# zifeo/distributed-sgd

Hardware: NVIDIA H100
Metric: sgd_samples_per_sec (higher is better)
Workload: dtype f64

## Files before the change

### distributed_sgd_b200/csrc/dsgd_fixed.cuh

```cuda
#pragma once
#include <cuda_runtime.h>
#include <stdint.h>

namespace dsgd {

constexpr int kAccStride = 16;
constexpr int kAccLimbs = 5;
constexpr int kAccWords = 2 * kAccLimbs + 1;
static_assert(kAccWords + 1 <= kAccStride, "acc_read loads the accumulator and one pad word");
__device__ __forceinline__ void red_add_u64(unsigned long long *p, unsigned long long v) {
  asm volatile("red.relaxed.gpu.global.add.u64 [%0], %1;" ::"l"(p), "l"(v) : "memory");
}
template <class Put>
__device__ __forceinline__ void acc_cut(double a, Put &&put) {
  double F[kAccLimbs - 1];
#pragma unroll
  for (int i = 0; i < kAccLimbs - 1; ++i) F[i] = floor(a * __longlong_as_double((1023ll + 40 * i) << 52));
  put(kAccLimbs - 1, F[0]);
#pragma unroll
  for (int i = 1; i < kAccLimbs - 1; ++i) put(kAccLimbs - 1 - i, F[i] - F[i - 1] * 0x1p40);
  put(0, rint(a * 0x1p160) - F[kAccLimbs - 2] * 0x1p40);
}
__device__ __forceinline__ void acc_push_one(unsigned long long *limbs, unsigned long long *ovf, double v) {
  if (!(fabs(v) < 4503599627370496.0)) {
    red_add_u64(ovf, 1ull);
    return;
  }
  const bool neg = v < 0.0;
  acc_cut(fabs(v), [&](int k, double limb) {
    if (limb != 0.0) {
      const unsigned long long u = (unsigned long long)(long long)limb;
      red_add_u64(limbs + k, neg ? (0ull - u) : u);
    }
  });
}
__device__ __forceinline__ void acc_push(unsigned long long *acc, double sd, double sn) {
  acc_push_one(acc, acc + 2 * kAccLimbs, sd);
  acc_push_one(acc + kAccLimbs, acc + 2 * kAccLimbs, sn);
}
__device__ __forceinline__ double acc_limb(unsigned long long q, int k) {
  return (double)(long long)q * __longlong_as_double((long long)(1023 - 160 + 40 * (k % kAccLimbs)) << 52);
}
__device__ __forceinline__ void acc_read(const unsigned long long *acc, int lane, double &sd, double &sn) {
  unsigned long long q0 = 0, q1 = 0;
  if (lane < (kAccWords + 1) / 2)
    asm volatile("ld.relaxed.gpu.global.v2.u64 {%0, %1}, [%2];" : "=l"(q0), "=l"(q1) : "l"(acc + 2 * lane) : "memory");
  const double lo = acc_limb(q0, 2 * lane), hi = acc_limb(q1, 2 * lane + 1), pair = lo + hi;
  const double s01 = __shfl_sync(0xffffffffu, pair, 0), s23 = __shfl_sync(0xffffffffu, pair, 1);
  const double s4 = __shfl_sync(0xffffffffu, lo, 2), n0 = __shfl_sync(0xffffffffu, hi, 2);
  const double n12 = __shfl_sync(0xffffffffu, pair, 3), n34 = __shfl_sync(0xffffffffu, pair, 4);
  sd = (s01 + s23) + s4;
  sn = (n0 + n12) + n34;
  if (__any_sync(0xffffffffu, lane == kAccWords / 2 && q0 != 0)) {
    sd = __longlong_as_double(0x7ff8000000000000ll);
    sn = sd;
  }
}

constexpr int kLossLimbs = kAccLimbs + 1;
constexpr int kLossAccWords = kLossLimbs + 1;
constexpr unsigned long long kLimbMask = (1ull << 40) - 1;
__device__ __forceinline__ void acc_carry(unsigned long long (&q)[kLossLimbs]) {
#pragma unroll
  for (int i = 0; i < kLossLimbs - 1; ++i) {
    q[i + 1] += q[i] >> 40;
    q[i] &= kLimbMask;
  }
}
__device__ __forceinline__ void acc_add_local(unsigned long long (&lim)[kLossLimbs], unsigned long long &ovf, double v) {
  if (!(v >= 0.0 && v < 4503599627370496.0)) { ++ovf; return; }
  acc_cut(v, [&](int k, double limb) { lim[k] += (unsigned long long)(long long)limb; });
  acc_carry(lim);
}
__device__ __forceinline__ void acc_flush_local(unsigned long long *acc, const unsigned long long (&lim)[kLossLimbs],
                                                unsigned long long ovf) {
#pragma unroll
  for (int i = 0; i < kLossLimbs; ++i)
    if (lim[i]) red_add_u64(acc + i, lim[i]);
  if (ovf) red_add_u64(acc + kLossLimbs, ovf);
}
__device__ __forceinline__ double acc_value(const unsigned long long *acc) {
  if (acc[kLossLimbs] != 0ull) return __longlong_as_double(0x7ff8000000000000ll);
  unsigned long long q[kLossLimbs];
#pragma unroll
  for (int i = 0; i < kLossLimbs; ++i) q[i] = acc[i];
  acc_carry(q);
  double s = (double)q[kLossLimbs - 1] * 0x1p40;
#pragma unroll
  for (int i = kLossLimbs - 2; i >= 0; --i) s += (double)q[i] * __longlong_as_double((long long)(1023 - 160 + 40 * i) << 52);
  return s;
}

}
```

### distributed_sgd_b200/csrc/dsgd_persistent.cuh

```cuda
#pragma once
#include <cuda_runtime.h>
#include <stdint.h>

#include "dsgd_fixed.cuh"
#include "dsgd_kernels.cuh"

namespace dsgd {

constexpr int kMaxWorld = 8;

struct PersistParams {
  const uint32_t *rp16;
  const uint2 *pairs;
  const int8_t *label;
  const int32_t *samples;
  int64_t n_steps;
  int32_t batch;
  int32_t dim;
  double *wbuf[2];
  double *gbuf[3];
  double2 *rec[3];
  const double *d;
  unsigned long long *acc;
  unsigned *hinge;
  double *losses;
  double *w_out;
  float *w32_out;
  double *scal;
  unsigned *bar;
  int *abort_flag;
  double lambda, lr, k_den;
  long long timeout_cycles;
  long long *tl;
  int world, rank;
  int64_t step_base;
  unsigned long long *xval[kMaxWorld];
  unsigned long long *xbm[kMaxWorld];
  int xstride, xwords;
  unsigned long long *llw[2];
  unsigned long long *xstats;
  double *avg;
};
static_assert(sizeof(PersistParams) <= 4000, "kernel parameter space is 4 KB");

__device__ __forceinline__ uint32_t smem_u32(const void *p) { return (uint32_t)__cvta_generic_to_shared(p); }
__device__ __forceinline__ void mbar_init(uint64_t *b, unsigned count) {
  asm volatile("mbarrier.init.shared::cta.b64 [%0], %1;" ::"r"(smem_u32(b)), "r"(count) : "memory");
}
__device__ __forceinline__ void mbar_expect_tx(uint64_t *b, unsigned bytes) {
  asm volatile("mbarrier.arrive.expect_tx.shared::cta.b64 _, [%0], %1;" ::"r"(smem_u32(b)), "r"(bytes) : "memory");
}
__device__ __forceinline__ void mbar_arrive(uint64_t *b) {
  asm volatile("mbarrier.arrive.shared::cta.b64 _, [%0];" ::"r"(smem_u32(b)) : "memory");
}
__device__ __forceinline__ void bulk_g2s(void *dst, const void *src, unsigned bytes, uint64_t *b) {
  asm volatile("cp.async.bulk.shared::cluster.global.mbarrier::complete_tx::bytes [%0], [%1], %2, [%3];" ::"r"(
                   smem_u32(dst)),
               "l"(src), "r"(bytes), "r"(smem_u32(b))
               : "memory");
}
__device__ __forceinline__ bool mbar_try_wait(uint64_t *b, unsigned parity) {
  unsigned ok;
  asm volatile(
      "{\n\t.reg .pred p;\n\tmbarrier.try_wait.parity.shared::cta.b64 p, [%1], %2;\n\tselp.u32 %0, 1, 0, p;\n\t}"
      : "=r"(ok)
      : "r"(smem_u32(b)), "r"(parity)
      : "memory");
  return ok != 0;
}
__device__ __forceinline__ void mbar_wait(uint64_t *b, unsigned parity, int *abort_flag, long long timeout) {
  if (mbar_try_wait(b, parity)) return;
  const long long t0 = clock64();
  unsigned spins = 0;
  while (!mbar_try_wait(b, parity)) {
    if ((++spins & 255u) == 0u && (clock64() - t0 > timeout || *(volatile int *)abort_flag)) {
      *(volatile int *)abort_flag = 1;
      return;
    }
  }
}
__device__ __forceinline__ unsigned ld_relaxed_gpu(const unsigned *p) {
  unsigned v;
  asm volatile("ld.relaxed.gpu.global.u32 %0, [%1];" : "=r"(v) : "l"(p) : "memory");
  return v;
}
__device__ __forceinline__ void red_release_gpu_add(unsigned *p, unsigned v) {
  asm volatile("red.release.gpu.global.add.u32 [%0], %1;" ::"l"(p), "r"(v) : "memory");
}
__device__ __forceinline__ unsigned atom_acq_rel_gpu_add(unsigned *p, unsigned v) {
  unsigned old;
  asm volatile("atom.acq_rel.gpu.global.add.u32 %0, [%1], %2;" : "=r"(old) : "l"(p), "r"(v) : "memory");
  return old;
}
__device__ __forceinline__ void st_relaxed_gpu(unsigned *p, unsigned v) {
  asm volatile("st.relaxed.gpu.global.u32 [%0], %1;" ::"l"(p), "r"(v) : "memory");
}
__device__ __forceinline__ void fence_acq_rel_gpu() { asm volatile("fence.acq_rel.gpu;" ::: "memory"); }
__device__ __forceinline__ void named_bar_sync(int id, int n_threads) {
  asm volatile("bar.sync %0, %1;" ::"r"(id), "r"(n_threads) : "memory");
}
__device__ __forceinline__ long long global_ns() {
  long long t;
  asm volatile("mov.u64 %0, %%globaltimer;" : "=l"(t));
  return t;
}

__device__ __forceinline__ void ll_store(unsigned long long *dst, double v, unsigned tag) {
  const unsigned long long bits = (unsigned long long)__double_as_longlong(v);
  const unsigned long long w0 = (bits & 0xffffffffull) | ((unsigned long long)tag << 32);
  const unsigned long long w1 = (bits >> 32) | ((unsigned long long)tag << 32);
  asm volatile("st.relaxed.sys.global.v2.u64 [%0], {%1, %2};" ::"l"(dst), "l"(w0), "l"(w1) : "memory");
}
__device__ __forceinline__ bool ll_try_load(const unsigned long long *src, unsigned tag, double &v) {
  unsigned long long w0, w1;
  asm volatile("ld.relaxed.sys.global.v2.u64 {%0, %1}, [%2];" : "=l"(w0), "=l"(w1) : "l"(src) : "memory");
  if ((unsigned)(w0 >> 32) != tag || (unsigned)(w1 >> 32) != tag) return false;
  v = __longlong_as_double((long long)((w0 & 0xffffffffull) | (w1 << 32)));
  return true;
}
__device__ __forceinline__ void ll_store32(unsigned long long *dst, unsigned v, unsigned tag) {
  const unsigned long long w = (unsigned long long)v | ((unsigned long long)tag << 32);
  asm volatile("st.relaxed.sys.global.u64 [%0], %1;" ::"l"(dst), "l"(w) : "memory");
}
__device__ __forceinline__ bool ll_try_load32(const unsigned long long *src, unsigned tag, unsigned &v) {
  unsigned long long w;
  asm volatile("ld.relaxed.sys.global.u64 %0, [%1];" : "=l"(w) : "l"(src) : "memory");
  v = (unsigned)w;
  return (unsigned)(w >> 32) == tag;
}

__device__ __forceinline__ double apply_update(double wv, double graw, double c, bool add_c, double k_den, double lr) {
  double v = filt(graw);
  if (v != 0.0) {
    if (add_c) v = filt(v + c);
    if (v != 0.0) {
      const double mean = (k_den == 1.0) ? v : filt(v / k_den);
      const double step = filt(mean * lr);
      wv = filt(wv - step);
    }
  }
  return wv;
}

__device__ __forceinline__ bool grid_barrier_arrive_wait(unsigned *bar, unsigned target, int *abort_flag, long long timeout) {
  red_release_gpu_add(bar, 1u);
  const long long t0 = clock64();
  unsigned spins = 0;
  bool ok = true;
  while ((int)(ld_relaxed_gpu(bar) - target) < 0) {
    if ((++spins & 1023u) == 0u && (clock64() - t0 > timeout || *(volatile int *)abort_flag)) {
      *(volatile int *)abort_flag = 1;
      ok = false;
      break;
    }
  }
  return ok;
}

constexpr int kChunkPairs = 128;
constexpr uint32_t kChunkGlobal = 1u << 31;
constexpr int kMaxRowsPerCta = 32;

template <int kMaxChunks>
struct StageMeta {
  int n_rows;
  int n_chunks;
  int n_multi;
  int n_pairs;
  int row_y[kMaxRowsPerCta];
  uint32_t row_b[kMaxRowsPerCta];
  int row_len[kMaxRowsPerCta];
  short row_first[kMaxRowsPerCta];
  short row_nch[kMaxRowsPerCta];
  uint32_t ch_off[kMaxChunks];
  short ch_n[kMaxChunks];
  short ch_row[kMaxChunks];
  double part[kMaxChunks];
};

template <int kCons, int kUpd, int kStages, int kStagePairs, int kMaxChunks>
struct PersistSmem {
  uint2 ring[kStages][kStagePairs];
  StageMeta<kMaxChunks> meta[kStages];
  uint64_t full[kStages];
  uint64_t empty[kStages];
  uint64_t c_bar[2];
  uint64_t u_bar;
  double red[kCons + kUpd][2];
  double c_val[2];
  double nrm_val[2];
  unsigned hinge_acc;
  int ok;
  long long tl_warp[kCons + kUpd];
};

#define DSGD_TL(slot_)                                                                        \
  do {                                                                                        \
    if (p.tl && blockIdx.x == 0 && lane == 0 && t < 256) p.tl[t * 16 + (slot_)] = clock64(); \
  } while (0)
constexpr int kTlSteps = 4, kTlFirst = 100, kTlCtas = 160, kTlPerCta = 4;
constexpr int kTlWords = 256 * 16 + kTlSteps * kTlCtas * kTlPerCta;

struct FetchLocal {
  const double2 *R;
  uint64_t *cbar;
  unsigned cpar;
  const double *cval;
  int *abort_flag;
  long long timeout;
  double k_den, lr;
  double c = 0.0;
  bool add_c = false, have_c = false, good = true;
  __device__ __forceinline__ void need_c() {
    if (!have_c) {
      mbar_wait(cbar, cpar, abort_flag, timeout);
      c = *(volatile const double *)cval;
      add_c = (c != 0.0) && (fabs(c) > kEps);
      have_c = true;
    }
  }
  __device__ __forceinline__ void get4(const uint2 (&pr)[4], double (&wv)[4]) {
    double2 r[4];
#pragma unroll
    for (int u = 0; u < 4; ++u) {
      r[u] = make_double2(0.0, 0.0);
      if (pr[u].y << 1) r[u] = __ldcg(&R[pr[u].x]);
    }
    need_c();
#pragma unroll
    for (int u = 0; u < 4; ++u) wv[u] = apply_update(r[u].x, r[u].y, c, add_c, k_den, lr);
  }
  __device__ __forceinline__ double get1(uint32_t col) {
    need_c();
    const double2 r = __ldcg(&R[col]);
    return apply_update(r.x, r.y, c, add_c, k_den, lr);
  }
};
struct FetchLL {
  const unsigned long long *LW;
  unsigned tag;
  int *abort_flag;
  long long timeout;
  bool good = true;
  __device__ __forceinline__ void spin(const unsigned long long *src, double &v) {
    unsigned spins = 0;
    const long long t0 = clock64();
    while (!ll_try_load(src, tag, v)) {
      if ((++spins & 255u) == 0u && (clock64() - t0 > timeout || *(volatile int *)abort_flag)) {
        *(volatile int *)abort_flag = 1;
        good = false;
        v = 0.0;
        break;
      }
    }
  }
  __device__ __forceinline__ void get4(const uint2 (&pr)[4], double (&wv)[4]) {
    unsigned pend = 0;
#pragma unroll
    for (int u = 0; u < 4; ++u) {
      wv[u] = 0.0;
      if (pr[u].y << 1) pend |= 1u << u;
    }
    unsigned spins = 0;
    const long long t0 = clock64();
    while (pend) {
      unsigned long long w0[4], w1[4];
#pragma unroll
      for (int u = 0; u < 4; ++u) {
        w0[u] = 0ull; w1[u] = 0ull;
        if (pend & (1u << u))
          asm volatile("ld.relaxed.sys.global.v2.u64 {%0, %1}, [%2];" : "=l"(w0[u]), "=l"(w1[u]) : "l"(LW + 2 * (size_t)pr[u].x) : "memory");
      }
#pragma unroll
      for (int u = 0; u < 4; ++u)
        if ((pend & (1u << u)) && (unsigned)(w0[u] >> 32) == tag && (unsigned)(w1[u] >> 32) == tag) {
          wv[u] = __longlong_as_double((long long)((w0[u] & 0xffffffffull) | (w1[u] << 32)));
          pend &= ~(1u << u);
        }
      if (pend && (++spins & 63u) == 0u && (clock64() - t0 > timeout || *(volatile int *)abort_flag)) {
        *(volatile int *)abort_flag = 1;
        good = false;
        pend = 0;
      }
    }
  }
  __device__ __forceinline__ double get1(uint32_t col) {
    double v;
    spin(LW + 2 * (size_t)col, v);
    return v;
  }
};

template <int kCons, int kMaxChunks, class Fetch>
__device__ __forceinline__ unsigned consume_stage(StageMeta<kMaxChunks> &mt, const uint2 *ring, const uint2 *pairs, double *gbase,
                                                  const int gstride, Fetch &fetch, int warp, int lane, long long *tl) {
  const int n_ch = mt.n_chunks;
  unsigned hinge = 0;
  for (int c = warp; c < n_ch; c += kCons) {
    const uint32_t off = mt.ch_off[c];
    const int n = mt.ch_n[c];
    const uint2 *src = (off & kChunkGlobal) ? (pairs + (off & ~kChunkGlobal)) : (ring + off);
    uint2 pr[4];
    double wv[4];
#pragma unroll
    for (int u = 0; u < 4; ++u) {
      const int k = u * 32 + lane;
      pr[u] = (k < n) ? src[k] : make_uint2(0u, 0u);
    }
    fetch.get4(pr, wv);
    double acc = 0.0;
#pragma unroll
    for (int u = 0; u < 4; ++u) acc += filt(filt((double)__uint_as_float(pr[u].y)) * wv[u]);
    if (tl && lane == 0 && c == warp) tl[2] = clock64();
    acc = warp_sum(acc);
    if (tl && lane == 0 && c == warp) tl[4] = clock64();
    {
      const int row1 = mt.ch_row[c];
      if (mt.row_nch[row1] == 1) {
        const int yi = mt.row_y[row1];
        const double y = (double)yi;
        if (lane == 0) hinge += (unsigned)(1 - yi * pred_of(acc));
        if (!(y * acc < 0.0)) {
#pragma unroll
          for (int u = 0; u < 4; ++u) {
            const double gvv = filt(filt((double)__uint_as_float(pr[u].y)) * y);
            if (gvv != 0.0) red_add_f64(gbase + (size_t)gstride * pr[u].x, gvv);
          }
        }
        continue;
      }
    }
    if (lane == 0) mt.part[c] = acc;
  }
  if (mt.n_multi > 0) {
    named_bar_sync(2, kCons * 32);
    for (int c = warp; c < n_ch; c += kCons) {
      const int row = mt.ch_row[c];
      const int first = mt.row_first[row], nch = mt.row_nch[row];
      if (nch == 1) continue;
      double dot = 0.0;
      for (int i = 0; i < nch; ++i) dot += mt.part[first + i];
      const int yi = mt.row_y[row];
      const double y = (double)yi;
      if (c == first && lane == 0) hinge += (unsigned)(1 - yi * pred_of(dot));
      if (!(y * dot < 0.0)) {
        const uint32_t off = mt.ch_off[c];
        const int n = mt.ch_n[c];
        const uint2 *src = (off & kChunkGlobal) ? (pairs + (off & ~kChunkGlobal)) : (ring + off);
        for (int k = lane; k < n; k += 32) {
          const uint2 pr = src[k];
          const double gvv = filt(filt((double)__uint_as_float(pr.y)) * y);
          if (gvv != 0.0) red_add_f64(gbase + (size_t)gstride * pr.x, gvv);
        }
      }
    }
  }
  for (int m = warp; m < mt.n_rows; m += kCons) {
    const int nch = mt.row_nch[m];
    if (nch == 0) {
      if (lane == 0) hinge += 1u;
    } else if (nch < 0) {
      const uint2 *grow = pairs + (size_t)mt.row_b[m] * 2;
      const int len = mt.row_len[m];
      double acc = 0.0;
      for (int k = lane; k < len; k += 32) {
        const uint2 pr = __ldg(&grow[k]);
        acc += filt(filt((double)__uint_as_float(pr.y)) * fetch.get1(pr.x));
      }
      const double dot = warp_sum(acc);
      const int yi = mt.row_y[m];
      const double y = (double)yi;
      if (lane == 0) hinge += (unsigned)(1 - yi * pred_of(dot));
      if (!(y * dot < 0.0))
        for (int k = lane; k < len; k += 32) {
          const uint2 pr = __ldg(&grow[k]);
          const double gvv = filt(filt((double)__uint_as_float(pr.y)) * y);
          if (gvv != 0.0) red_add_f64(gbase + (size_t)gstride * pr.x, gvv);
        }
    }
  }
  return hinge;
}

template <int kCons, int kUpd, int kStages, int kStagePairs, int kMaxChunks, bool kMulti, bool kAvg>
__global__ void __launch_bounds__((kCons + kUpd + 1) * 32, 1) k_sync_persistent(const PersistParams p) {
  using Smem = PersistSmem<kCons, kUpd, kStages, kStagePairs, kMaxChunks>;
  extern __shared__ __align__(128) unsigned char smem_raw[];
  Smem &sm = *reinterpret_cast<Smem *>(smem_raw);

  const int lane = threadIdx.x & 31;
  const int warp = threadIdx.x >> 5;
  const bool is_cons = warp < kCons;
  const bool is_upd = warp >= kCons && warp < kCons + kUpd;
  const int G = gridDim.x;
  const int B = p.batch;
  const int64_t S = p.n_steps;
  constexpr int kSyncThreads = (kCons + kUpd) * 32;
  const int n_r = (B > (int)blockIdx.x) ? (B - 1 - (int)blockIdx.x) / G + 1 : 0;

  if (threadIdx.x == 0) {
    for (int s = 0; s < kStages; ++s) {
      mbar_init(&sm.full[s], 1u);
      mbar_init(&sm.empty[s], (unsigned)kCons);
    }
    mbar_init(&sm.c_bar[0], 1u);
    mbar_init(&sm.c_bar[1], 1u);
    mbar_init(&sm.u_bar, (unsigned)(kMulti ? kCons + kUpd : kUpd));
    sm.c_val[0] = 0.0;
    sm.nrm_val[0] = 0.0;
    sm.hinge_acc = 0u;
    sm.ok = 1;
  }
  asm volatile("fence.mbarrier_init.release.cluster;" ::: "memory");
  __syncthreads();
  if (threadIdx.x == 0) mbar_arrive(&sm.c_bar[0]);

  if (!is_cons && !is_upd) {
    auto load_id = [&](int64_t t) -> int32_t {
      return (t < S && lane < n_r) ? __ldg(&p.samples[t * B + blockIdx.x + lane * G]) : -1;
    };
    uint32_t b0 = 0, e0 = 0, b1 = 0, e1 = 0;
    int y0 = 0, y1 = 0;
    auto load_win = [&](int32_t id, uint32_t &b, uint32_t &e, int &y) {
      b = 0u; e = 0u; y = 0;
      if (id >= 0) {
        b = __ldg(&p.rp16[id]);
        e = __ldg(&p.rp16[id + 1]);
        y = (int)__ldg(&p.label[id]);
      }
    };
    load_win(load_id(0), b0, e0, y0);
    load_win(load_id(1), b1, e1, y1);
    int32_t id_next = load_id(2);
    for (int64_t t = 0; t < S; ++t) {
      const int st = (int)t & (kStages - 1);
      if (t >= kStages) {
        mbar_wait(&sm.empty[st], (unsigned)(((t / kStages) - 1) & 1), p.abort_flag, p.timeout_cycles);
        if (*(volatile int *)p.abort_flag) return;
      }
      auto &mt = sm.meta[st];
      const int len = (lane < n_r) ? (int)(e0 - b0) * 2 : 0;
      const int nch = (len + kChunkPairs - 1) / kChunkPairs;
      int ps = len, cs = nch;
#pragma unroll
      for (int o = 1; o < 32; o <<= 1) {
        const int a = __shfl_up_sync(0xffffffffu, ps, o), c2 = __shfl_up_sync(0xffffffffu, cs, o);
        if (lane >= o) { ps += a; cs += c2; }
      }
      const int my_pair = ps - len, my_chunk = cs - nch;
      const bool listed = (my_chunk + nch) <= kMaxChunks;
      const bool in_ring = listed && (my_pair + len) <= kStagePairs;
      if (lane < n_r) {
        mt.row_y[lane] = y0;
        mt.row_b[lane] = b0;
        mt.row_len[lane] = len;
        mt.row_first[lane] = (short)my_chunk;
        mt.row_nch[lane] = (short)(listed ? nch : -1);
        if (listed) {
          for (int c = 0; c < nch; ++c) {
            const int n = min(kChunkPairs, len - c * kChunkPairs);
            mt.ch_off[my_chunk + c] = in_ring ? (uint32_t)(my_pair + c * kChunkPairs)
                                              : (kChunkGlobal | (b0 * 2u + (uint32_t)(c * kChunkPairs)));
            mt.ch_n[my_chunk + c] = (short)n;
            mt.ch_row[my_chunk + c] = (short)lane;
          }
        }
      }
      const unsigned my_bytes = (lane < n_r && in_ring) ? (unsigned)len * 8u : 0u;
      const unsigned ring_bytes = __reduce_add_sync(0xffffffffu, my_bytes);
      const int listed_chunks = __reduce_max_sync(0xffffffffu, (lane < n_r && listed) ? (my_chunk + nch) : 0);
      const unsigned multi = __ballot_sync(0xffffffffu, lane < n_r && listed && nch > 1);
      if (lane == 31) mt.n_pairs = ps;
      if (lane == 0) {
        mt.n_rows = n_r;
        mt.n_chunks = listed_chunks;
        mt.n_multi = __popc(multi);
      }
      __syncwarp();
      if (lane == 0) {
        if (ring_bytes) mbar_expect_tx(&sm.full[st], ring_bytes);
        else mbar_arrive(&sm.full[st]);
      }
      __syncwarp();
      if (my_bytes) bulk_g2s(&sm.ring[st][my_pair], p.pairs + (size_t)b0 * 2, my_bytes, &sm.full[st]);
      b0 = b1; e0 = e1; y0 = y1;
      load_win(id_next, b1, e1, y1);
      id_next = load_id(t + 3);
    }
    return;
  }

  const double lr = p.lr;
  const int64_t base = kMulti ? p.step_base : 0;
  unsigned phase = 0;
  const int n_upd = G * kUpd * 32;
  const int u0 = blockIdx.x * kUpd * 32 + ((int)threadIdx.x - kCons * 32);
  const int K = p.world, me = p.rank;
  const int slice = ((p.dim + 1 + G - 1) / G + 31) & ~31;
  const int j_col = blockIdx.x * slice + (int)threadIdx.x;
  const bool col_act = kMulti && (int)threadIdx.x < slice && j_col <= p.dim;
  const int col_word = j_col >> 5;
  unsigned long long st_val = 0, st_bm = 0;
  constexpr int kUpdCols = 2;
  double wreg[kUpdCols], dreg[kUpdCols];
  double areg[kUpdCols];
  int ttl[kUpdCols];
  bool gnz[kUpdCols];
#pragma unroll
  for (int i = 0; i < kUpdCols; ++i) {
    wreg[i] = dreg[i] = 0.0;
    areg[i] = 0.0;
    ttl[i] = 0;
    gnz[i] = false;
    if constexpr (!kMulti) {
      const int j = u0 + i * n_upd;
      if (is_upd && j < p.dim) {
        wreg[i] = __ldcg(&p.rec[2][j].x);
        dreg[i] = __ldg(&p.d[j]);
        if constexpr (kAvg) areg[i] = p.avg[j];
      }
    }
  }
  if constexpr (kMulti) {
    if (col_act && j_col < p.dim) {
      wreg[0] = __ldcg(&p.wbuf[0][j_col]);
      dreg[0] = __ldg(&p.d[j_col]);
      if constexpr (kAvg) areg[0] = p.avg[j_col];
    }
  }

  int gi_prev = (int)((base + 2) % 3), gi_cur = (int)(base % 3), gi_next = (int)((base + 1) % 3);
  int ti_prev = 2, ti_cur = 0, ti_next = 1;
  for (int64_t T = base; T <= base + S; ++T) {
    const int64_t t = T - base;
    const bool first = (t == 0), last = (t == S);
    const double *Gprev = p.gbuf[gi_prev];
    double *Gcur = p.gbuf[gi_cur];
    double *Gzero = p.gbuf[gi_next];
    const unsigned long long *acc_prev = p.acc + (size_t)ti_prev * kAccStride;
    unsigned long long *acc_cur = p.acc + (size_t)ti_cur * kAccStride;
    unsigned long long *acc_next = p.acc + (size_t)ti_next * kAccStride;
    const double2 *Rprev = p.rec[ti_prev];
    double2 *Rcur = p.rec[ti_cur];
    double2 *Rnext = p.rec[ti_next];
    const unsigned c_par = (unsigned)((t >> 1) & 1);
    const bool tl_cta = p.tl && t >= kTlFirst && t < kTlFirst + kTlSteps && blockIdx.x < kTlCtas;
    long long *tl_rec = tl_cta ? p.tl + 256 * 16 + ((t - kTlFirst) * kTlCtas + blockIdx.x) * kTlPerCta : nullptr;
    long long *tl_row = (p.tl && blockIdx.x == 0 && t < 256) ? p.tl + t * 16 : nullptr;
    bool ok = true;
    if (warp == 0) DSGD_TL(0);

    if (warp == kCons && !first) {
      double c_prev, nrm_prev;
      if (kMulti && t == 1) {
        c_prev = p.scal[kScalC];
        nrm_prev = p.scal[kScalNrm2];
      } else {
        double sd, sn;
        acc_read(acc_prev, lane, sd, sn);
        c_prev = p.lambda * 2.0 * sd;
        nrm_prev = sn;
      }
      if (blockIdx.x == 0 && lane < kAccWords) acc_next[lane] = 0ull;
      if (lane == 0) {
        sm.c_val[t & 1] = c_prev;
        sm.nrm_val[t & 1] = nrm_prev;
        mbar_arrive(&sm.c_bar[t & 1]);
        if (!kMulti && p.losses && blockIdx.x == 0)
          p.losses[t - 1] = p.lambda * nrm_prev + (double)__ldcg(&p.hinge[t - 1]) / (double)B;
      }
      __syncwarp();
      DSGD_TL(9);
    }
    double pd = 0.0, pn = 0.0;
    auto publish_partial = [&]() {
      pd = warp_sum(pd);
      pn = warp_sum(pn);
      if (lane == 0) {
        sm.red[warp][0] = pd;
        sm.red[warp][1] = pn;
        mbar_arrive(&sm.u_bar);
      }
      if (warp == kCons) {
        mbar_wait(&sm.u_bar, (unsigned)(t & 1), p.abort_flag, p.timeout_cycles);
        if (lane == 0) {
          double sd = 0.0, sn = 0.0;
#pragma unroll
          for (int i = kMulti ? 0 : kCons; i < kCons + kUpd; ++i) { sd += sm.red[i][0]; sn += sm.red[i][1]; }
          if (sd != 0.0 || sn != 0.0) acc_push(acc_cur, sd, sn);
        }
        __syncwarp();
      }
    };

    if constexpr (kMulti) {
      unsigned long long *LWcur = p.llw[T & 1];
      const int parp = (int)((T + 1) & 1);
      const unsigned gtag = (unsigned)T;
      const unsigned wtag = (unsigned)(T + 1);
      if ((int)threadIdx.x < slice) {
        if (first) {
          if (col_act) {
            if (j_col < p.dim) ll_store(LWcur + 2 * (size_t)j_col, wreg[0], wtag);
            Gzero[j_col] = 0.0;
          }
        } else {
          double own = 0.0;
          if (col_act) {
            own = __ldcg(&Gprev[j_col]);
            if (j_col < p.dim) own = filt(own);
          }
          const unsigned my_bits = __ballot_sync(0xffffffffu, own != 0.0);
          const bool warp_act = blockIdx.x * slice + (warp << 5) <= p.dim;
          if (warp_act) {
            const size_t vslot = 2 * (((size_t)me * 2 + parp) * p.xstride + (size_t)j_col);
            const size_t bslot = ((size_t)me * 2 + parp) * p.xwords + (size_t)col_word;
            for (int k = 0; k < K; ++k) {
              if (k == me) continue;
              if (lane == 0) ll_store32(p.xbm[k] + bslot, my_bits, gtag);
              if (own != 0.0) ll_store(p.xval[k] + vslot, own, gtag);
            }
            if (lane == 0) { st_bm += 1; st_val += (unsigned)__popc(my_bits); }
          }
          if (warp == 0) DSGD_TL(11);
          if (warp_act) {
            double raw[kMaxWorld];
            unsigned need = 0;
            double wn = wreg[0];
            const unsigned long long *bm0 = p.xbm[me] + (size_t)parp * p.xwords + (size_t)col_word;
            const unsigned long long *vl0 = p.xval[me] + 2 * ((size_t)parp * p.xstride + (size_t)j_col);
            unsigned bits[kMaxWorld];
            unsigned pend = 0;
#pragma unroll
            for (int k = 0; k < kMaxWorld; ++k) {
              raw[k] = (k == me) ? own : 0.0;
              bits[k] = 0u;
              if (k < K && k != me) pend |= 1u << k;
            }
            {
              unsigned spins = 0;
              const long long t0 = clock64();
              while (pend) {
#pragma unroll
                for (int k = 0; k < kMaxWorld; ++k)
                  if (pend & (1u << k)) {
                    if (ll_try_load32(bm0 + (size_t)k * 2 * p.xwords, gtag, bits[k])) pend &= ~(1u << k);
                  }
                if (pend && (++spins & 63u) == 0u && (clock64() - t0 > p.timeout_cycles || *(volatile int *)p.abort_flag)) {
                  *(volatile int *)p.abort_flag = 1;
                  ok = false;
#pragma unroll
                  for (int k = 0; k < kMaxWorld; ++k)
                    if (pend & (1u << k)) bits[k] = 0u;
                  pend = 0;
                }
              }
            }
#pragma unroll
            for (int k = 0; k < kMaxWorld; ++k)
              if (k < K && k != me && ((bits[k] >> lane) & 1u)) need |= 1u << k;
            auto poll_values = [&]() {
              unsigned long long v0[kMaxWorld], v1[kMaxWorld];
#pragma unroll
              for (int k = 0; k < kMaxWorld; ++k) {
                v0[k] = 0ull; v1[k] = 0ull;
                if (need & (1u << k))
                  asm volatile("ld.relaxed.sys.global.v2.u64 {%0, %1}, [%2];"
                               : "=l"(v0[k]), "=l"(v1[k]) : "l"(vl0 + 2 * (size_t)k * 2 * p.xstride) : "memory");
              }
#pragma unroll
              for (int k = 0; k < kMaxWorld; ++k)
                if ((need & (1u << k)) && (unsigned)(v0[k] >> 32) == gtag && (unsigned)(v1[k] >> 32) == gtag) {
                  raw[k] = __longlong_as_double((long long)((v0[k] & 0xffffffffull) | (v1[k] << 32)));
                  need &= ~(1u << k);
                }
            };
            if (need) poll_values();
            mbar_wait(&sm.c_bar[t & 1], c_par, p.abort_flag, p.timeout_cycles);
            const double c_prev = *(volatile double *)&sm.c_val[t & 1];
            const bool add_c = (c_prev != 0.0) && (fabs(c_prev) > kEps);
            if (col_act) {
              {
                unsigned spins = 0;
                const long long t0 = clock64();
                while (need) {
                  poll_values();
                  if (need && (++spins & 63u) == 0u && (clock64() - t0 > p.timeout_cycles || *(volatile int *)p.abort_flag)) {
                    *(volatile int *)p.abort_flag = 1;
                    ok = false;
                    need = 0;
                  }
                }
              }
              double s = 0.0;
#pragma unroll
              for (int k = 0; k < kMaxWorld; ++k) {
                if (k < K) {
                  if (j_col == p.dim) {
                    s += raw[k];
                  } else {
                    double v = filt(raw[k]);
                    if (v != 0.0 && add_c) v = filt(v + c_prev);
                    s = (k == 0) ? v : filt(s + v);
                  }
                }
              }
              if (j_col == p.dim) {
                if (p.losses) {
                  const double ns = floor(s / 4294967296.0);
                  p.losses[t - 1] = p.lambda * *(volatile double *)&sm.nrm_val[t & 1] + (s - ns * 4294967296.0) / ns;
                }
              } else {
                if (s != 0.0) {
                  const double mean = filt(s / (double)K);
                  const double step = filt(mean * lr);
                  wn = filt(wn - step);
                }
                wreg[0] = wn;
                if constexpr (kAvg) areg[0] = areg[0] + wn;
                ll_store(LWcur + 2 * (size_t)j_col, wn, wtag);
                pd = filt(wn * dreg[0]);
                pn = wn * wn;
              }
              Gzero[j_col] = 0.0;
            }
          }
        }
      }
      if (warp == 0) DSGD_TL(12);
      publish_partial();
      if (is_cons && !last) {
        const int st = (int)t & (kStages - 1);
        auto &mt = sm.meta[st];
        mbar_wait(&sm.full[st], (unsigned)(((unsigned)t / kStages) & 1u), p.abort_flag, p.timeout_cycles);
        if (warp == 0) DSGD_TL(1);
        FetchLL fetch{LWcur, wtag, p.abort_flag, p.timeout_cycles};
        const unsigned hinge = consume_stage<kCons, kMaxChunks>(mt, &sm.ring[st][0], p.pairs, Gcur, 1, fetch, warp, lane,
                                                                          warp == 0 ? tl_row : nullptr);
        ok = ok && fetch.good;
        if (lane == 0 && hinge) atomicAdd(&sm.hinge_acc, hinge);
        if (tl_rec && warp == 0 && lane == 0) tl_rec[2] = mt.n_pairs;
        __syncwarp();
        if (lane == 0) mbar_arrive(&sm.empty[st]);
        if (warp == 0) DSGD_TL(3);
      }
    } else {
      if (is_cons) {
        if (!last) {
          const int st = (int)t & (kStages - 1);
          auto &mt = sm.meta[st];
          mbar_wait(&sm.full[st], (unsigned)(((unsigned)t / kStages) & 1u), p.abort_flag, p.timeout_cycles);
          if (warp == 0) DSGD_TL(1);
          FetchLocal fetch{Rprev, &sm.c_bar[t & 1], c_par, &sm.c_val[t & 1], p.abort_flag, p.timeout_cycles, p.k_den, lr};
          const unsigned hinge = consume_stage<kCons, kMaxChunks>(mt, &sm.ring[st][0], p.pairs, &Rcur[0].y, 2, fetch, warp,
                                                                            lane, warp == 0 ? tl_row : nullptr);
          if (lane == 0 && hinge) atomicAdd(&sm.hinge_acc, hinge);
          if (tl_rec && warp == 0 && lane == 0) tl_rec[2] = mt.n_pairs;
          __syncwarp();
          if (lane == 0) mbar_arrive(&sm.empty[st]);
          if (warp == 0) DSGD_TL(3);
        }
      } else {
        double gv[kUpdCols];
#pragma unroll
        for (int i = 0; i < kUpdCols; ++i) {
          const int j = u0 + i * n_upd;
          gv[i] = (j < p.dim) ? __ldcg(&Rprev[j].y) : 0.0;
        }
        mbar_wait(&sm.c_bar[t & 1], c_par, p.abort_flag, p.timeout_cycles);
        const double c_prev = *(volatile double *)&sm.c_val[t & 1];
        const bool add_c = (c_prev != 0.0) && (fabs(c_prev) > kEps);
#pragma unroll
        for (int i = 0; i < kUpdCols; ++i) {
          const int j = u0 + i * n_upd;
          if (j < p.dim) {
            if (gv[i] != 0.0) {
              wreg[i] = apply_update(wreg[i], gv[i], c_prev, add_c, p.k_den, lr);
              ttl[i] = 3;
            }
            if (ttl[i] > 0) { Rcur[j].x = wreg[i]; --ttl[i]; }
            if (gnz[i]) Rnext[j].y = 0.0;
            gnz[i] = gv[i] != 0.0;
            if constexpr (kAvg) if (!first) areg[i] = areg[i] + wreg[i];
            pd += filt(wreg[i] * dreg[i]);
            pn += wreg[i] * wreg[i];
          }
        }
        for (int j = u0 + kUpdCols * n_upd; j < p.dim; j += n_upd) {
          const double2 r = __ldcg(&Rprev[j]);
          const double wn = apply_update(r.x, r.y, c_prev, add_c, p.k_den, lr);
          Rcur[j].x = wn;
          Rnext[j].y = 0.0;
          if constexpr (kAvg) if (!first) p.avg[j] = p.avg[j] + wn;
          pd += filt(wn * __ldg(&p.d[j]));
          pn += wn * wn;
        }
        if (warp == kCons) DSGD_TL(10);
        publish_partial();
      }
    }

    if (!ok) *(volatile int *)&sm.ok = 0;
    if (tl_row && lane == 0) sm.tl_warp[warp] = clock64();
    named_bar_sync(3, kSyncThreads);
    ++phase;
    if (threadIdx.x == 0) {
      if (tl_row) {
        long long mc = 0, mu = 0;
        for (int i = 0; i < kCons; ++i) mc = max(mc, sm.tl_warp[i]);
        for (int i = kCons; i < kCons + kUpd; ++i) mu = max(mu, sm.tl_warp[i]);
        tl_row[13] = mc;
        tl_row[14] = mu;
      }
      if (!last) {
        const unsigned h = sm.hinge_acc;
        if constexpr (kMulti) {
          if (h) red_add_f64(&Gcur[p.dim], (double)h);
          if (blockIdx.x == 0) red_add_f64(&Gcur[p.dim], (double)B * 4294967296.0);
        } else {
          if (h) atomicAdd(&p.hinge[t], h);
        }
        sm.hinge_acc = 0u;
      }
      if (tl_rec) tl_rec[0] = global_ns();
      else if (tl_row) tl_row[6] = clock64();
      bool bar_ok = grid_barrier_arrive_wait(p.bar, phase * (unsigned)G, p.abort_flag, p.timeout_cycles);
      if (*(volatile int *)&sm.ok == 0) { *(volatile int *)p.abort_flag = 1; bar_ok = false; }
      sm.ok = bar_ok ? 1 : 0;
      if (tl_rec) tl_rec[1] = global_ns();
      else if (tl_row) tl_row[7] = clock64();
    }
    named_bar_sync(3, kSyncThreads);
    if (*(volatile int *)&sm.ok == 0) return;
    { const int a = gi_prev; gi_prev = gi_cur; gi_cur = gi_next; gi_next = a; }
    { const int a = ti_prev; ti_prev = ti_cur; ti_cur = ti_next; ti_next = a; }
  }

  if (blockIdx.x == 0 && warp == kCons && S > 0) {
    double sd, sn;
    acc_read(p.acc + (size_t)ti_prev * kAccStride, lane, sd, sn);
    if (lane == 0) { p.scal[kScalC] = p.lambda * 2.0 * sd; p.scal[kScalNrm2] = sn; }
  }
  if constexpr (kMulti) {
    const unsigned long long *LW = p.llw[(base + S) & 1];
    const unsigned wtag = (unsigned)(base + S + 1);
    const int n_all = G * kSyncThreads;
    for (int j = blockIdx.x * kSyncThreads + threadIdx.x; j < p.dim; j += n_all) {
      double wv = 0.0;
      ll_try_load(LW + 2 * (size_t)j, wtag, wv);
      p.w_out[j] = wv;
      p.w32_out[j] = (float)wv;
    }
    if (p.xstats && lane == 0 && (st_val | st_bm)) {
      atomicAdd(&p.xstats[0], st_val);
      atomicAdd(&p.xstats[1], st_bm);
    }
    if constexpr (kAvg) {
      if (col_act && j_col < p.dim) p.avg[j_col] = areg[0];
    }
  } else if (is_upd) {
    const double2 *Rfin = p.rec[ti_prev];
#pragma unroll
    for (int i = 0; i < kUpdCols; ++i) {
      const int j = u0 + i * n_upd;
      if (j < p.dim) {
        p.w_out[j] = wreg[i];
        p.w32_out[j] = (float)wreg[i];
        if constexpr (kAvg) p.avg[j] = areg[i];
      }
    }
    for (int j = u0 + kUpdCols * n_upd; j < p.dim; j += n_upd) {
      const double wv = __ldcg(&Rfin[j]).x;
      p.w_out[j] = wv;
      p.w32_out[j] = (float)wv;
    }
  }
}

__global__ void __launch_bounds__(256) k_rec_init(const double *__restrict__ w, int dim, double2 *__restrict__ rec0,
                                                  double2 *__restrict__ rec1, double2 *__restrict__ rec2) {
  const int j = blockIdx.x * blockDim.x + threadIdx.x;
  if (j < dim) {
    const double2 r = make_double2(w[j], 0.0);
    rec0[j] = r;
    rec1[j] = r;
    rec2[j] = r;
  }
}

}
```

Baseline: 70.19 million.

## Spread accumulator pushes across warp lanes and overlap loss write with barrier

The fixed-point accumulator push is now done by eleven lanes in parallel, each computing and atomically adding one limb, where a single lane used to issue up to eleven serial reductions. The single-GPU loss record is moved out of the consumer warp's critical path and into the grid-barrier wait, and the barrier issues its first poll before running that side work. The update warps' gradient loads are hoisted to the top of the step so they are in flight earlier. In exchange, every lane recomputes the full limb cut and each update thread keeps more live registers.

After: 70.57 million, median of 6. About the same (+0.5%).

```diff
diff --git a/distributed_sgd_b200/csrc/dsgd_fixed.cuh b/distributed_sgd_b200/csrc/dsgd_fixed.cuh
--- a/distributed_sgd_b200/csrc/dsgd_fixed.cuh
+++ b/distributed_sgd_b200/csrc/dsgd_fixed.cuh
@@ -21,22 +21,22 @@
   for (int i = 1; i < kAccLimbs - 1; ++i) put(kAccLimbs - 1 - i, F[i] - F[i - 1] * 0x1p40);
   put(0, rint(a * 0x1p160) - F[kAccLimbs - 2] * 0x1p40);
 }
-__device__ __forceinline__ void acc_push_one(unsigned long long *limbs, unsigned long long *ovf, double v) {
-  if (!(fabs(v) < 4503599627370496.0)) {
-    red_add_u64(ovf, 1ull);
-    return;
+__device__ __forceinline__ bool acc_overflows(double v) { return !(fabs(v) < 4503599627370496.0); }
+__device__ __forceinline__ void acc_push(unsigned long long *acc, int lane, double sd, double sn) {
+  unsigned long long u = 0ull;
+  if (lane < 2 * kAccLimbs) {
+    const double v = lane < kAccLimbs ? sd : sn;
+    const int my = lane % kAccLimbs;
+    if (!acc_overflows(v)) {
+      double mine = 0.0;
+      acc_cut(fabs(v), [&](int k, double limb) { if (k == my) mine = limb; });
+      u = (unsigned long long)(long long)mine;
+      if (v < 0.0) u = 0ull - u;
+    }
+  } else if (lane == 2 * kAccLimbs) {
+    u = (unsigned long long)acc_overflows(sd) + (unsigned long long)acc_overflows(sn);
   }
-  const bool neg = v < 0.0;
-  acc_cut(fabs(v), [&](int k, double limb) {
-    if (limb != 0.0) {
-      const unsigned long long u = (unsigned long long)(long long)limb;
-      red_add_u64(limbs + k, neg ? (0ull - u) : u);
-    }
-  });
-}
-__device__ __forceinline__ void acc_push(unsigned long long *acc, double sd, double sn) {
-  acc_push_one(acc, acc + 2 * kAccLimbs, sd);
-  acc_push_one(acc + kAccLimbs, acc + 2 * kAccLimbs, sn);
+  if (u != 0ull) red_add_u64(acc + lane, u);
 }
 __device__ __forceinline__ double acc_limb(unsigned long long q, int k) {
   return (double)(long long)q * __longlong_as_double((long long)(1023 - 160 + 40 * (k % kAccLimbs)) << 52);
diff --git a/distributed_sgd_b200/csrc/dsgd_persistent.cuh b/distributed_sgd_b200/csrc/dsgd_persistent.cuh
--- a/distributed_sgd_b200/csrc/dsgd_persistent.cuh
+++ b/distributed_sgd_b200/csrc/dsgd_persistent.cuh
@@ -142,17 +142,22 @@
   return wv;
 }
 
-__device__ __forceinline__ bool grid_barrier_arrive_wait(unsigned *bar, unsigned target, int *abort_flag, long long timeout) {
+template <class Meanwhile>
+__device__ __forceinline__ bool grid_barrier_arrive_wait(unsigned *bar, unsigned target, int *abort_flag, long long timeout,
+                                                         Meanwhile &&meanwhile) {
   red_release_gpu_add(bar, 1u);
+  unsigned seen = ld_relaxed_gpu(bar);
+  meanwhile();
   const long long t0 = clock64();
   unsigned spins = 0;
   bool ok = true;
-  while ((int)(ld_relaxed_gpu(bar) - target) < 0) {
+  while ((int)(seen - target) < 0) {
     if ((++spins & 1023u) == 0u && (clock64() - t0 > timeout || *(volatile int *)abort_flag)) {
       *(volatile int *)abort_flag = 1;
       ok = false;
       break;
     }
+    seen = ld_relaxed_gpu(bar);
   }
   return ok;
 }
@@ -550,6 +555,17 @@
     bool ok = true;
     if (warp == 0) DSGD_TL(0);
 
+    double gv[kUpdCols];
+    if constexpr (!kMulti) {
+      if (is_upd) {
+#pragma unroll
+        for (int i = 0; i < kUpdCols; ++i) {
+          const int j = u0 + i * n_upd;
+          gv[i] = (j < p.dim) ? __ldcg(&Rprev[j].y) : 0.0;
+        }
+      }
+    }
+
     if (warp == kCons && !first) {
       double c_prev, nrm_prev;
       if (kMulti && t == 1) {
@@ -566,8 +582,6 @@
         sm.c_val[t & 1] = c_prev;
         sm.nrm_val[t & 1] = nrm_prev;
         mbar_arrive(&sm.c_bar[t & 1]);
-        if (!kMulti && p.losses && blockIdx.x == 0)
-          p.losses[t - 1] = p.lambda * nrm_prev + (double)__ldcg(&p.hinge[t - 1]) / (double)B;
       }
       __syncwarp();
       DSGD_TL(9);
@@ -583,12 +597,10 @@
       }
       if (warp == kCons) {
         mbar_wait(&sm.u_bar, (unsigned)(t & 1), p.abort_flag, p.timeout_cycles);
-        if (lane == 0) {
-          double sd = 0.0, sn = 0.0;
-#pragma unroll
-          for (int i = kMulti ? 0 : kCons; i < kCons + kUpd; ++i) { sd += sm.red[i][0]; sn += sm.red[i][1]; }
-          if (sd != 0.0 || sn != 0.0) acc_push(acc_cur, sd, sn);
-        }
+        double sd = 0.0, sn = 0.0;
+#pragma unroll
+        for (int i = kMulti ? 0 : kCons; i < kCons + kUpd; ++i) { sd += sm.red[i][0]; sn += sm.red[i][1]; }
+        acc_push(acc_cur, lane, sd, sn);
         __syncwarp();
       }
     };
@@ -761,12 +773,6 @@
           if (warp == 0) DSGD_TL(3);
         }
       } else {
-        double gv[kUpdCols];
-#pragma unroll
-        for (int i = 0; i < kUpdCols; ++i) {
-          const int j = u0 + i * n_upd;
-          gv[i] = (j < p.dim) ? __ldcg(&Rprev[j].y) : 0.0;
-        }
         mbar_wait(&sm.c_bar[t & 1], c_par, p.abort_flag, p.timeout_cycles);
         const double c_prev = *(volatile double *)&sm.c_val[t & 1];
         const bool add_c = (c_prev != 0.0) && (fabs(c_prev) > kEps);
@@ -824,7 +830,10 @@
       }
       if (tl_rec) tl_rec[0] = global_ns();
       else if (tl_row) tl_row[6] = clock64();
-      bool bar_ok = grid_barrier_arrive_wait(p.bar, phase * (unsigned)G, p.abort_flag, p.timeout_cycles);
+      bool bar_ok = grid_barrier_arrive_wait(p.bar, phase * (unsigned)G, p.abort_flag, p.timeout_cycles, [&] {
+        if (!kMulti && p.losses && blockIdx.x == 0 && !first)
+          p.losses[t - 1] = p.lambda * sm.nrm_val[t & 1] + (double)__ldcg(&p.hinge[t - 1]) / (double)B;
+      });
       if (*(volatile int *)&sm.ok == 0) { *(volatile int *)p.abort_flag = 1; bar_ok = false; }
       sm.ok = bar_ok ? 1 : 0;
       if (tl_rec) tl_rec[1] = global_ns();
```
